# meyerls/FruitNeRF

Hardware: AMD Instinct MI355X
Metric: train rays/sec, fruit_nerf on synthetic apple 800x800 (higher is better)
Workload: dtype f32 fwd (MLP GEMMs: 3-piece bf16 split, 6 products, ~2^-24) / 2-piece bwd (dX, dW: 3 products, ~2^-17; its forward recompute 3-piece); everything else f32

## Files before the change

### fruitnerf_amd/csrc/hash_sources.hpp

```cpp
#pragma once
#include "common.hpp"

namespace fnr {

struct RaySource {
  RaysDev rays;
  const float* euclid;
  int S;
  __device__ __forceinline__ void position(long long n, float& px, float& py, float& pz) const {
    long long r = n / S;
    int k = (int)(n - r * S);
    const float* b = euclid + r * (S + 1) + k;
    ray_position(rays.origins + 3 * r, rays.directions + 3 * r, b[0], b[1], px, py, pz);
  }
};

struct LatticeSource {
  const float* xs;
  const float* ys;
  const float* zs;
  int n_y, n_z;
  long long ray_begin;
  __device__ __forceinline__ void position(long long n, float& px, float& py, float& pz) const {
    long long r = n / n_z;
    int k = (int)(n - r * n_z);
    r += ray_begin;
    long long ix = r / n_y;
    int iy = (int)(r - ix * n_y);
    px = xs[ix];
    py = ys[iy];
    pz = zs[k];
  }
};

__device__ __forceinline__ void blend_input_grad(const float (&d)[8], const float (&o)[3], float (&g)[3]) {
  const float ox = o[0], oy = o[1], oz = o[2];
  const float mx = 1.0f - ox, my = 1.0f - oy, mz = 1.0f - oz;
  g[0] = oz * (oy * (d[0] - d[3]) + my * (d[1] - d[2])) + mz * (oy * (d[4] - d[7]) + my * (d[5] - d[6]));
  g[1] = oz * (ox * (d[0] - d[1]) + mx * (d[3] - d[2])) + mz * (ox * (d[4] - d[5]) + mx * (d[7] - d[6]));
  g[2] = oy * (ox * (d[0] - d[4]) + mx * (d[3] - d[7])) + my * (ox * (d[1] - d[5]) + mx * (d[2] - d[6]));
}

__device__ __forceinline__ void decode_block(int b, int L, long long nsb, int& level, long long& sb) {
  if ((L & 7) == 0) {
    const int xcd = b & 7;
    const long long q = b >> 3;
    const int li = (int)(q / nsb);
    sb = q - (long long)li * nsb;
    const int base = (li >> 1) * 8 + xcd;
    level = (li & 1) ? (L - 1 - base) : base;
  } else {
    level = b % L;
    sb = b / L;
  }
}

}
```

### fruitnerf_amd/csrc/hashgrid.hip

```cpp
#include <type_traits>

#include "hash_sources.hpp"
#include "sequencer.hpp"

namespace fnr {

constexpr int ENC_SPT = 2;

template <class Source>
__global__ __launch_bounds__(256) void k_hash_encode(GridDev grid, Warp warp, Source src, long long N,
                                                     float2* __restrict__ feats, uint8_t* __restrict__ selector,
                                                     float2* __restrict__ jac) {
  const long long nsb = (N + 256 * ENC_SPT - 1) / (256 * ENC_SPT);
  int level;
  long long sb;
  decode_block(blockIdx.x, grid.n_levels, nsb, level, sb);
  const uint32_t mask = (1u << grid.log2_T) - 1u;
  const float2* lt = grid.table + ((size_t)level << grid.log2_T);
  const int scaling = grid.scalings[level];
  uint32_t h[ENC_SPT][8];
  float o[ENC_SPT][3];
  bool sel[ENC_SPT];
  long long n[ENC_SPT];
#pragma unroll
  for (int u = 0; u < ENC_SPT; ++u) {
    n[u] = sb * (256 * ENC_SPT) + u * 256 + threadIdx.x;
    const long long nn = n[u] < N ? n[u] : N - 1;
    float px, py, pz, x[3];
    src.position(nn, px, py, pz);
    sel[u] = warp_position(warp, px, py, pz, x);
    const GridLevel g = grid_cell(x, scaling);
    grid_corners(g, mask, h[u]);
    o[u][0] = g.o[0], o[u][1] = g.o[1], o[u][2] = g.o[2];
  }
  const bool odd = threadIdx.x & 1;
  PairedRows rows[ENC_SPT];
#pragma unroll
  for (int u = 0; u < ENC_SPT; ++u) rows[u] = paired_rows(h[u], odd);
  float2 va[ENC_SPT][4], vb[ENC_SPT][4];
#pragma unroll
  for (int u = 0; u < ENC_SPT; ++u) {
#pragma unroll
    for (int j = 0; j < 4; ++j) va[u][j] = lt[rows[u].a[j]];
#pragma unroll
    for (int j = 0; j < 4; ++j) vb[u][j] = lt[rows[u].b[j]];
  }
  float2 v[ENC_SPT][8];
#pragma unroll
  for (int u = 0; u < ENC_SPT; ++u) paired_values(va[u], vb[u], odd, v[u]);
#pragma unroll
  for (int u = 0; u < ENC_SPT; ++u) {
    if (n[u] >= N) continue;
    feats[(size_t)level * N + n[u]] = grid_interp(v[u], o[u]);
    if (level == 0 && selector) selector[n[u]] = sel[u] ? 1 : 0;
    if (jac) {
      float dx[8], dy[8], gx[3], gy[3];
#pragma unroll
      for (int k = 0; k < 8; ++k) dx[k] = v[u][k].x, dy[k] = v[u][k].y;
      blend_input_grad(dx, o[u], gx);
      blend_input_grad(dy, o[u], gy);
      const float s = sel[u] ? (float)scaling : 0.0f;
#pragma unroll
      for (int a = 0; a < 3; ++a) ntc_store<NT_JAC_ST>(&jac[((size_t)level * 3 + a) * N + n[u]], make_float2(s * gx[a], s * gy[a]));
    }
  }
}

template <class Source>
static int launch_encode(const fnr_grid* grid, const fnr_warp* warp, const Source& src, long long N, float* feats,
                         uint8_t* selector, float* jacobian, void* stream) {
  FNR_CHECK_ARG(grid && warp && feats, "hash_encode: null argument");
  FNR_CHECK_ARG(grid->n_levels >= 1 && grid->n_levels <= FNR_MAX_LEVELS, "hash_encode: n_levels %d out of range",
                grid->n_levels);
  FNR_CHECK_ARG(grid->log2_hashmap_size >= 1 && grid->log2_hashmap_size <= 28, "hash_encode: log2_hashmap_size");
  if (N == 0) return FNR_OK;
  const long long nsb = (N + 256 * ENC_SPT - 1) / (256 * ENC_SPT);
  const long long nblk = nsb * grid->n_levels;
  FNR_CHECK_ARG(nblk < (1ll << 31), "hash_encode: too many samples for one launch (%lld)", N);
  constexpr int prof_op = std::is_same<Source, LatticeSource>::value ? OP_ENCODE_LATTICE : OP_ENCODE_FWD;
  FNR_PROF(prof_op, N);
  hipLaunchKernelGGL((k_hash_encode<Source>), dim3((unsigned)nblk), dim3(256), 0, as_stream(stream), make_grid(grid),
                     make_warp(warp), src, N, reinterpret_cast<float2*>(feats), selector,
                     reinterpret_cast<float2*>(jacobian));
  FNR_LAUNCH_CHECK();
  return FNR_OK;
}

template <int L, int H>
__global__ __launch_bounds__(256) void k_prop_density(GridDev grid, Warp warp, RaySource src, long long N,
                                                      const float* __restrict__ w0, const float* __restrict__ b0,
                                                      const float* __restrict__ w1, const float* __restrict__ b1,
                                                      float* __restrict__ density, float2* __restrict__ feat_save) {
  const long long n = (long long)blockIdx.x * 256 + threadIdx.x;
  if (n >= N) return;
  float px, py, pz, x[3];
  src.position(n, px, py, pz);
  const bool sel = warp_position(warp, px, py, pz, x);
  const uint32_t mask = (1u << grid.log2_T) - 1u;
  float f[2 * L];
#pragma unroll
  for (int l = 0; l < L; ++l) {
    float2 v = grid_lookup(grid.table + ((size_t)l << grid.log2_T), x, grid.scalings[l], mask);
    f[2 * l] = v.x;
    f[2 * l + 1] = v.y;
    if (feat_save) ntc_store<NT_PROP_FEATS>(&feat_save[(size_t)l * N + n], v);
  }
  float out = b1[0];
#pragma unroll
  for (int o = 0; o < H; ++o) {
    float a = b0[o];
#pragma unroll
    for (int k = 0; k < 2 * L; ++k) a = fmaf(w0[o * 2 * L + k], f[k], a);
    a = fmaxf(a, 0.0f);
    out = fmaf(w1[o], a, out);
  }
  density[n] = sel ? expf(out) : 0.0f;
}

}

using namespace fnr;

extern "C" int fnr_hash_encode_fwd(const fnr_grid* grid, const fnr_warp* warp, const fnr_rays* rays,
                                   const float* euclid_bins, int S, float* feats, uint8_t* selector, float* jacobian,
                                   void* stream) {
  if (seq::recording() && grid && warp && rays) {
    const fnr_grid grid_ = *grid;
    const fnr_warp warp_ = *warp;
    const fnr_rays rays_ = *rays;
    seq::push("fnr_hash_encode_fwd", [=](const fnr_step_scalars*) {
      return fnr_hash_encode_fwd(&grid_, &warp_, &rays_, euclid_bins, S, feats, selector, jacobian, stream);
    });
  }
  FNR_CHECK_ARG(rays && euclid_bins && S > 0, "hash_encode_fwd: null rays/bins or S<=0");
  RaySource src{make_rays(rays), euclid_bins, S};
  return launch_encode(grid, warp, src, rays->n_rays * (long long)S, feats, selector, jacobian, stream);
}

extern "C" int fnr_hash_encode_lattice(const fnr_grid* grid, const fnr_warp* warp, const fnr_lattice* lat,
                                       int64_t ray_begin, int64_t n_rays, float* feats, uint8_t* selector,
                                       void* stream) {
  FNR_SEQ_UNRECORDABLE("fnr_hash_encode_lattice");
  FNR_CHECK_ARG(lat && lat->xs && lat->ys && lat->zs, "hash_encode_lattice: null lattice");
  FNR_CHECK_ARG(ray_begin >= 0 && n_rays >= 0 && ray_begin + n_rays <= (int64_t)lat->n_x * lat->n_y,
                "hash_encode_lattice: ray range [%lld,+%lld) outside %d x %d lattice", (long long)ray_begin,
                (long long)n_rays, lat->n_x, lat->n_y);
  LatticeSource src{lat->xs, lat->ys, lat->zs, lat->n_y, lat->n_z, ray_begin};
  return launch_encode(grid, warp, src, n_rays * (long long)lat->n_z, feats, selector, nullptr, stream);
}

extern "C" int fnr_prop_density_fwd(const fnr_prop_net* net, const fnr_warp* warp, const fnr_rays* rays,
                                    const float* euclid_bins, int S, float* density, float* feat_save, void* stream) {
  if (seq::recording() && net && warp && rays) {
    const fnr_prop_net net_ = *net;
    const fnr_warp warp_ = *warp;
    const fnr_rays rays_ = *rays;
    seq::push("fnr_prop_density_fwd", [=](const fnr_step_scalars*) {
      return fnr_prop_density_fwd(&net_, &warp_, &rays_, euclid_bins, S, density, feat_save, stream);
    });
  }
  FNR_CHECK_ARG(net && warp && rays && euclid_bins && density && S > 0, "prop_density_fwd: null argument");
  FNR_UNSUPPORTED(net->hidden_dim == 16, "prop_density_fwd: hidden_dim %d not built (16 only)", net->hidden_dim);
  const long long N = rays->n_rays * (long long)S;
  if (N == 0) return FNR_OK;
  RaySource src{make_rays(rays), euclid_bins, S};
  const unsigned nblk = (unsigned)((N + 255) / 256);
  GridDev g = make_grid(&net->grid);
  Warp w = make_warp(warp);
  float2* fs = reinterpret_cast<float2*>(feat_save);
  FNR_PROF(OP_PROP_FWD, N);
#define FNR_PROP_CASE(LL)                                                                                      \
  case LL:                                                                                                     \
    hipLaunchKernelGGL((k_prop_density<LL, 16>), dim3(nblk), dim3(256), 0, as_stream(stream), g, w, src, N,    \
                       net->w0, net->b0, net->w1, net->b1, density, fs);                                       \
    break;
  switch (net->grid.n_levels) {
    FNR_PROP_CASE(1)
    FNR_PROP_CASE(2)
    FNR_PROP_CASE(3)
    FNR_PROP_CASE(4)
    FNR_PROP_CASE(5)
    FNR_PROP_CASE(6)
    FNR_PROP_CASE(7)
    FNR_PROP_CASE(8)
    default:
      FNR_UNSUPPORTED(false, "prop_density_fwd: n_levels %d not built (1..8)", net->grid.n_levels);
  }
#undef FNR_PROP_CASE
  FNR_LAUNCH_CHECK();
  return FNR_OK;
}
```

Before: 6.492 million.

## Place hash-encode blocks on XCDs by per-level L2 footprint cost

```diff
diff --git a/fruitnerf_amd/csrc/encode_placement.hpp b/fruitnerf_amd/csrc/encode_placement.hpp
--- /dev/null
+++ b/fruitnerf_amd/csrc/encode_placement.hpp
@@ -0,0 +1,128 @@
+#pragma once
+
+#if defined(__HIPCC__) || defined(__CUDACC__)
+#define FNR_PLACEMENT_HD __host__ __device__
+#else
+#define FNR_PLACEMENT_HD
+#endif
+
+namespace fnr {
+
+constexpr int ENC_XCDS = 8;
+constexpr int ENC_MAX_SEGMENTS = 8;
+constexpr int ENC_MAX_PLACED_LEVELS = 64;
+constexpr long long ENC_L2_SMALL_BYTES = 1ll << 20, ENC_L2_FIT_BYTES = 2ll << 20;
+constexpr int ENC_COST_SMALL = 4, ENC_COST_FIT = 5;
+constexpr int ENC_COST_FILL_2 = 6, ENC_COST_FILL_4 = 7, ENC_COST_FILL_16 = 8, ENC_COST_FULL = 9;
+
+struct EncodePlacement {
+  int seg_q0[ENC_XCDS][ENC_MAX_SEGMENTS];
+  int seg_first[ENC_XCDS][ENC_MAX_SEGMENTS];
+  int seg_level[ENC_XCDS][ENC_MAX_SEGMENTS];
+  int n_seg[ENC_XCDS];
+  int run_blocks[ENC_XCDS];
+};
+
+inline long long encode_lattice_rows(int scaling) {
+  const long long r = (long long)scaling + 1;
+  return r > 1000000 ? (1ll << 60) : r * r * r;
+}
+inline int encode_level_cost(int scaling, int log2_T) {
+  const long long T = 1ll << log2_T, dense = encode_lattice_rows(scaling);
+  const long long bytes = 8 * (dense < T ? dense : T);
+  if (bytes <= ENC_L2_SMALL_BYTES) return ENC_COST_SMALL;
+  if (bytes <= ENC_L2_FIT_BYTES) return ENC_COST_FIT;
+  if (dense < 2 * T) return ENC_COST_FILL_2;
+  if (dense < 4 * T) return ENC_COST_FILL_4;
+  if (dense < 16 * T) return ENC_COST_FILL_16;
+  return ENC_COST_FULL;
+}
+
+inline void encode_cut_levels(int l0, int l1, long long nsb, const int* cost, const long long* num, long long den, long long* cut) {
+  typedef __int128 wide;
+  long long prefix[ENC_MAX_PLACED_LEVELS + 1];
+  prefix[l0] = 0;
+  for (int l = l0; l < l1; ++l) prefix[l + 1] = prefix[l] + nsb * cost[l];
+  const long long C = prefix[l1];
+  cut[0] = l0 * nsb;
+  cut[ENC_XCDS] = l1 * nsb;
+  for (int k = 1; k < ENC_XCDS; ++k) {
+    if (l1 == l0 || den <= 0) {
+      cut[k] = (num[k] >= den) ? cut[ENC_XCDS] : cut[0];
+      continue;
+    }
+    int l = l0;
+    while (l + 1 < l1 && (wide)den * prefix[l + 1] <= (wide)num[k] * C) ++l;
+    const wide w = cost[l];
+    wide j = (2 * ((wide)num[k] * C - (wide)den * prefix[l]) + den * w) / (2 * den * w);
+    if (j < 0) j = 0;
+    if (j > nsb) j = nsb;
+    cut[k] = l * nsb + (long long)j;
+    if (cut[k] < cut[k - 1]) cut[k] = cut[k - 1];
+  }
+}
+
+inline long long encode_partition(int L, long long nsb, const int* cost, EncodePlacement& out) {
+  if (L < 1 || L > ENC_MAX_PLACED_LEVELS || nsb < 1 || nsb * L >= (1ll << 31)) return 0;
+  for (int l = 0; l < L; ++l)
+    if (cost[l] < 1 || cost[l] > 1024) return 0;
+  int split = 0;
+  while (split < L && cost[split] < ENC_COST_FULL) ++split;
+  long long load[ENC_XCDS] = {}, q[ENC_XCDS] = {}, total = 0;
+  for (int x = 0; x < ENC_XCDS; ++x) out.n_seg[x] = 0;
+  for (int l = 0; l < L; ++l) total += nsb * cost[l];
+  bool placed[ENC_MAX_PLACED_LEVELS] = {};
+  for (int i = 0; i < split; ++i) {
+    int l = -1, x = 0;
+    for (int c = 0; c < split; ++c)
+      if (!placed[c] && (l < 0 || cost[c] > cost[l])) l = c;
+    for (int c = 1; c < ENC_XCDS; ++c)
+      if (load[c] < load[x]) x = c;
+    placed[l] = true;
+    const int s = out.n_seg[x]++;
+    if (s == ENC_MAX_SEGMENTS) return 0;
+    out.seg_q0[x][s] = (int)q[x];
+    out.seg_first[x][s] = 0;
+    out.seg_level[x][s] = l;
+    q[x] += nsb;
+    load[x] += nsb * cost[l];
+  }
+  long long num[ENC_XCDS + 1], cut[ENC_XCDS + 1];
+  num[0] = 0;
+  for (int x = 0; x < ENC_XCDS; ++x) num[x + 1] = num[x] + (total > ENC_XCDS * load[x] ? total - ENC_XCDS * load[x] : 0);
+  encode_cut_levels(split, L, nsb, cost, num, num[ENC_XCDS], cut);
+  long long longest = 0;
+  for (int x = 0; x < ENC_XCDS; ++x) {
+    long long g = cut[x];
+    const long long end = cut[x + 1];
+    while (g < end) {
+      const int s = out.n_seg[x]++;
+      if (s == ENC_MAX_SEGMENTS) return 0;
+      const long long level = g / nsb, first = g - level * nsb;
+      const long long count = (end - g < nsb - first) ? end - g : nsb - first;
+      out.seg_q0[x][s] = (int)q[x];
+      out.seg_first[x][s] = (int)first;
+      out.seg_level[x][s] = (int)level;
+      g += count;
+      q[x] += count;
+    }
+    out.run_blocks[x] = (int)q[x];
+    for (int s = out.n_seg[x]; s < ENC_MAX_SEGMENTS; ++s) out.seg_q0[x][s] = out.seg_first[x][s] = out.seg_level[x][s] = 0;
+    if (q[x] > longest) longest = q[x];
+  }
+  if (longest * ENC_XCDS >= (1ll << 31)) return 0;
+  return longest;
+}
+
+FNR_PLACEMENT_HD inline bool placement_lookup(const EncodePlacement& P, int b, int& level, long long& sb) {
+  const int xcd = b & (ENC_XCDS - 1), q = b >> 3;
+  if (q >= P.run_blocks[xcd]) return false;
+  int s = 0;
+  for (int t = 1; t < ENC_MAX_SEGMENTS; ++t)
+    if (t < P.n_seg[xcd] && q >= P.seg_q0[xcd][t]) s = t;
+  level = P.seg_level[xcd][s];
+  sb = (long long)P.seg_first[xcd][s] + (q - P.seg_q0[xcd][s]);
+  return true;
+}
+
+}
diff --git a/fruitnerf_amd/csrc/hash_sources.hpp b/fruitnerf_amd/csrc/hash_sources.hpp
--- a/fruitnerf_amd/csrc/hash_sources.hpp
+++ b/fruitnerf_amd/csrc/hash_sources.hpp
@@ -1,5 +1,6 @@
 #pragma once
 #include "common.hpp"
+#include "encode_placement.hpp"
 
 namespace fnr {
 
@@ -55,4 +56,11 @@
   }
 }
 
+__device__ __forceinline__ bool decode_block(const EncodePlacement& P, int placed, int b, int L, long long nsb, int& level,
+                                             long long& sb) {
+  if (placed) return placement_lookup(P, b, level, sb);
+  decode_block(b, L, nsb, level, sb);
+  return true;
 }
+
+}
diff --git a/fruitnerf_amd/csrc/hashgrid.hip b/fruitnerf_amd/csrc/hashgrid.hip
--- a/fruitnerf_amd/csrc/hashgrid.hip
+++ b/fruitnerf_amd/csrc/hashgrid.hip
@@ -10,11 +10,11 @@
 template <class Source>
 __global__ __launch_bounds__(256) void k_hash_encode(GridDev grid, Warp warp, Source src, long long N,
                                                      float2* __restrict__ feats, uint8_t* __restrict__ selector,
-                                                     float2* __restrict__ jac) {
+                                                     float2* __restrict__ jac, int placed, EncodePlacement placement) {
   const long long nsb = (N + 256 * ENC_SPT - 1) / (256 * ENC_SPT);
   int level;
   long long sb;
-  decode_block(blockIdx.x, grid.n_levels, nsb, level, sb);
+  if (!decode_block(placement, placed, blockIdx.x, grid.n_levels, nsb, level, sb)) return;
   const uint32_t mask = (1u << grid.log2_T) - 1u;
   const float2* lt = grid.table + ((size_t)level << grid.log2_T);
   const int scaling = grid.scalings[level];
@@ -75,13 +75,26 @@
   FNR_CHECK_ARG(grid->log2_hashmap_size >= 1 && grid->log2_hashmap_size <= 28, "hash_encode: log2_hashmap_size");
   if (N == 0) return FNR_OK;
   const long long nsb = (N + 256 * ENC_SPT - 1) / (256 * ENC_SPT);
-  const long long nblk = nsb * grid->n_levels;
+  long long nblk = nsb * grid->n_levels;
   FNR_CHECK_ARG(nblk < (1ll << 31), "hash_encode: too many samples for one launch (%lld)", N);
+  EncodePlacement placement = {};
+  int placed = 0;
+#ifndef FNR_ENCODE_FIXED_PLACEMENT
+  if ((grid->n_levels & 7) == 0 && !std::is_same<Source, LatticeSource>::value) {
+    int cost[FNR_MAX_LEVELS];
+    for (int l = 0; l < grid->n_levels; ++l) cost[l] = encode_level_cost(grid->scalings[l], grid->log2_hashmap_size);
+    const long long longest = encode_partition(grid->n_levels, nsb, cost, placement);
+    if (longest > 0) {
+      placed = 1;
+      nblk = longest * ENC_XCDS;
+    }
+  }
+#endif
   constexpr int prof_op = std::is_same<Source, LatticeSource>::value ? OP_ENCODE_LATTICE : OP_ENCODE_FWD;
   FNR_PROF(prof_op, N);
   hipLaunchKernelGGL((k_hash_encode<Source>), dim3((unsigned)nblk), dim3(256), 0, as_stream(stream), make_grid(grid),
                      make_warp(warp), src, N, reinterpret_cast<float2*>(feats), selector,
-                     reinterpret_cast<float2*>(jacobian));
+                     reinterpret_cast<float2*>(jacobian), placed, placement);
   FNR_LAUNCH_CHECK();
   return FNR_OK;
 }
```

After: 6.450 million. No clear change (-0.7%).
